# LoganWilliams1/mhm2_kmer_analysis_v2

Hardware: AMD Instinct MI355X
Metric: k-mers/sec (kcount stage) at k=21 (higher is better)
Workload: dtype u64

## Files before the change

### include/kcount_mi355.h

```cpp
#ifndef KCOUNT_MI355_H
#define KCOUNT_MI355_H

#include <stddef.h>
#include <stdint.h>

#ifdef __cplusplus
extern "C" {
#endif

#define KC_ABI_VERSION 1

enum {
  KC_OK = 0,
  KC_ERR_INVALID_ARG = -1,
  KC_ERR_UNSUPPORTED_K = -2,
  KC_ERR_NO_DEVICE = -3,
  KC_ERR_HIP = -4,
  KC_ERR_OUT_OF_MEMORY = -5,
  KC_ERR_CAPACITY = -6,
  KC_ERR_BAD_BASE = -7,
  KC_ERR_STATE = -8
};

typedef struct kc_ctx kc_ctx;
// ... 16 lines not shown
#define KC_FLAG_SHARD_BUCKETS 4u
#define KC_FLAG_WIRE_UNITS 8u
#define KC_FLAG_TIME_KERNELS 1u

typedef struct kc_stats {
  uint64_t num_reads;
  uint64_t num_bases;
  uint64_t raw_kmers;
  uint64_t kmers_inserted;
  uint64_t num_unique;
  uint64_t num_purged;
  uint64_t total_kmers;
  uint64_t sum_counts;
  uint64_t num_dropped;
  uint64_t capacity;
  uint64_t num_gpu_calls;
  uint64_t table_bytes;
} kc_stats;

typedef struct kc_result {
  uint64_t n;
  int32_t num_longs;
  int32_t reserved;
  const uint64_t *d_keys;
  const uint16_t *d_counts;
  const uint8_t *d_left;
  const uint8_t *d_right;
} kc_result;

int kc_abi_version(void);
const char *kc_error_string(int status);
const char *kc_last_error(void);
int kc_device_count(void);

int kc_num_longs(int kmer_len);
int kc_record_longs(int kmer_len);
int kc_owner(const uint64_t *kmer_words, int kmer_len, int rank_n);
int kc_owner_reference(const uint64_t *kmer_words, int kmer_len, int rank_n);

kc_ctx *kc_create(const kc_config *cfg, int *status);
void kc_destroy(kc_ctx *ctx);
int kc_set_stream(kc_ctx *ctx, void *hip_stream);
int kc_reset(kc_ctx *ctx, int new_kmer_len);

int kc_submit_reads(kc_ctx *ctx, const uint8_t *bases, const uint8_t *quals, const uint64_t *offsets, uint64_t nreads,
                    int on_device);

int kc_submit_packed_reads(kc_ctx *ctx, const uint8_t *packed, const uint64_t *offsets, uint64_t nreads, int on_device);

int kc_fastq_to_packed(const char *text, uint64_t len, int qual_offset, uint8_t *packed, uint64_t packed_capacity, uint64_t *offsets,
                       uint64_t reads_capacity, uint64_t *nreads, uint64_t *nbytes);

int kc_fastq_pairs(const char *text1, uint64_t len1, const char *text2, uint64_t len2, uint8_t *bases, uint8_t *quals,
                   uint64_t capacity, uint64_t *offsets, uint64_t reads_capacity, uint64_t *nreads, uint64_t *nbytes);

#define KC_FASTQ_PARTIAL 1u

int kc_fastq_to_packed_device(kc_ctx *ctx, const char *text, uint64_t len, int on_device, uint32_t flags, uint8_t *d_packed,
                              uint64_t packed_capacity, uint64_t *d_offsets, uint64_t reads_capacity, uint64_t *nreads,
                              uint64_t *nbytes, uint64_t *consumed);

int kc_fastq_pairs_device(kc_ctx *ctx, const char *text1, uint64_t len1, const char *text2, uint64_t len2, int on_device,
                          uint32_t flags, uint8_t *d_bases, uint8_t *d_quals, uint64_t capacity, uint64_t *d_offsets,
                          uint64_t reads_capacity, uint64_t *nreads, uint64_t *nbytes, uint64_t *consumed1, uint64_t *consumed2);

typedef struct kc_merge_stats {
// ... 132 lines not shown
```

### mhm2_kmer_analysis_v2_amd/_lib.py

```python
import ctypes as C
import os

_HERE = os.path.dirname(os.path.abspath(__file__))
_LIB = None

KC_OK = 0
KC_ERR_INVALID_ARG = -1
KC_ERR_CAPACITY = -6
KC_ERR_UNSUPPORTED_K = -2
KC_ERR_BAD_BASE = -7
KC_ERR_STATE = -8
KC_FLAG_TIME_KERNELS = 1
KC_FASTQ_PARTIAL = 1
KC_ADAPTERS_BLASTN_SCORES = 1
KC_TRIM_PAIRED = 1
KC_FLAG_REFERENCE_OWNER = 2
KC_FLAG_SHARD_BUCKETS = 4
KC_FLAG_WIRE_UNITS = 8


class KcError(RuntimeError):
    def __init__(self, status, where=""):
        self.status = status
        L = lib()
# ... 19 lines not shown
                ("d_counts", C.c_void_p), ("d_left", C.c_void_p), ("d_right", C.c_void_p)]


class kc_tuning(C.Structure):
    _fields_ = [("mode", C.c_uint32), ("writers", C.c_uint32), ("p1", C.c_uint32), ("p2", C.c_uint32), ("slots", C.c_uint32),
                ("chunk1", C.c_uint32), ("chunk2", C.c_uint32), ("chain1_max", C.c_uint32), ("chain2_max", C.c_uint32),
                ("arena1", C.c_uint32), ("ovf_capacity", C.c_uint64)]


class kc_kernel_time(C.Structure):
    _fields_ = [("name", C.c_char * 48), ("launches", C.c_uint64), ("total_ms", C.c_double)]


class kc_synth_params(C.Structure):
    _fields_ = [("seed", C.c_uint64), ("num_genomes", C.c_uint32), ("read_len", C.c_uint32), ("min_genome_len", C.c_uint64),
                ("max_genome_len", C.c_uint64), ("sub_error_rate", C.c_double), ("lowq_rate", C.c_double),
                ("n_rate", C.c_double), ("abundance_sigma", C.c_double)]


class kc_merge_stats(C.Structure):
    _fields_ = [(n, C.c_uint64) for n in ("pairs", "merged", "ambiguous", "dropped", "overlap_len", "merged_len", "out_reads",
                                           "out_bases")]


class kc_trim_stats(C.Structure):
    _fields_ = [(n, C.c_uint64) for n in ("reads", "trimmed", "bases_trimmed", "reads_removed", "alignments", "out_bases")]


SYMBOLS = {
    "kc_abi_version": (C.c_int, []),
    "kc_error_string": (C.c_char_p, [C.c_int]),
    "kc_last_error": (C.c_char_p, []),
    "kc_device_count": (C.c_int, []),
    "kc_num_longs": (C.c_int, [C.c_int]),
    "kc_record_longs": (C.c_int, [C.c_int]),
    "kc_owner": (C.c_int, [C.c_void_p, C.c_int, C.c_int]),
    "kc_owner_reference": (C.c_int, [C.c_void_p, C.c_int, C.c_int]),
    "kc_create": (C.c_void_p, [C.POINTER(kc_config), C.POINTER(C.c_int)]),
    "kc_destroy": (None, [C.c_void_p]),
    "kc_set_stream": (C.c_int, [C.c_void_p, C.c_void_p]),
    "kc_reset": (C.c_int, [C.c_void_p, C.c_int]),
    "kc_submit_reads": (C.c_int, [C.c_void_p, C.c_void_p, C.c_void_p, C.c_void_p, C.c_uint64, C.c_int]),
    "kc_submit_packed_reads": (C.c_int, [C.c_void_p, C.c_void_p, C.c_void_p, C.c_uint64, C.c_int]),
    "kc_fastq_to_packed": (C.c_int, [C.c_char_p, C.c_uint64, C.c_int, C.c_void_p, C.c_uint64, C.c_void_p, C.c_uint64, C.POINTER(C.c_uint64),
                                      C.POINTER(C.c_uint64)]),
    "kc_fastq_pairs": (C.c_int, [C.c_char_p, C.c_uint64, C.c_char_p, C.c_uint64, C.c_void_p, C.c_void_p, C.c_uint64, C.c_void_p,
                                  C.c_uint64, C.POINTER(C.c_uint64), C.POINTER(C.c_uint64)]),
    "kc_fastq_to_packed_device": (C.c_int, [C.c_void_p, C.c_void_p, C.c_uint64, C.c_int, C.c_uint32, C.c_void_p, C.c_uint64, C.c_void_p,
                                             C.c_uint64, C.POINTER(C.c_uint64), C.POINTER(C.c_uint64), C.POINTER(C.c_uint64)]),
    "kc_fastq_pairs_device": (C.c_int, [C.c_void_p, C.c_void_p, C.c_uint64, C.c_void_p, C.c_uint64, C.c_int, C.c_uint32, C.c_void_p,
                                         C.c_void_p, C.c_uint64, C.c_void_p, C.c_uint64, C.POINTER(C.c_uint64), C.POINTER(C.c_uint64),
                                         C.POINTER(C.c_uint64), C.POINTER(C.c_uint64)]),
    "kc_merge_pairs": (C.c_int, [C.c_void_p, C.c_void_p, C.c_void_p, C.c_void_p, C.c_uint64, C.c_int, C.c_int, C.c_void_p, C.c_uint64,
                                  C.c_void_p, C.c_uint64, C.POINTER(C.c_uint64), C.POINTER(C.c_uint64), C.POINTER(kc_merge_stats)]),
    "kc_adapters_index": (C.c_int, [C.c_char_p, C.c_uint64, C.c_int, C.POINTER(C.c_uint64), C.POINTER(C.c_uint64), C.POINTER(C.c_uint64),
                                     C.POINTER(C.c_uint64)]),
    "kc_adapters_load": (C.c_int, [C.c_void_p, C.c_char_p, C.c_uint64, C.c_int, C.c_uint32, C.POINTER(C.c_uint64), C.POINTER(C.c_uint64),
                                    C.POINTER(C.c_uint64), C.POINTER(C.c_uint64)]),
    "kc_adapters_clear": (C.c_int, [C.c_void_p]),
    "kc_trim_adapters": (C.c_int, [C.c_void_p, C.c_void_p, C.c_void_p, C.c_void_p, C.c_uint64, C.c_int, C.c_uint32, C.c_void_p, C.c_void_p,
                                    C.c_uint64, C.c_void_p, C.POINTER(C.c_uint64), C.POINTER(kc_trim_stats)]),
    "kc_submit_seq_block": (C.c_int, [C.c_void_p, C.c_void_p, C.c_uint64, C.c_int]),
    "kc_extract_partition": (C.c_int, [C.c_void_p, C.c_void_p, C.c_void_p, C.c_void_p, C.c_uint64, C.c_int, C.c_void_p,
                                       C.c_uint64, C.c_void_p]),
    "kc_extract_partition_seq_block": (C.c_int, [C.c_void_p, C.c_void_p, C.c_uint64, C.c_int, C.c_void_p, C.c_uint64, C.c_void_p]),
    "kc_insert_records": (C.c_int, [C.c_void_p, C.c_void_p, C.c_uint64]),
# ... 57 lines not shown
```

### mhm2_kmer_analysis_v2_amd/csrc/kc_api.hip

```cpp
#include <hip/hip_runtime.h>

#include <math.h>
#include <stdio.h>
#include <stdlib.h>
#include <string.h>

#include <algorithm>
#include <new>
#include <thread>
#include <string>
#include <type_traits>
#include <unordered_map>
#include <vector>

#include "../../include/kcount_mi355.h"
#include "kc_bucketed.hpp"
#include "kc_shard.hpp"
#include "kc_wire6.hpp"
#include "kc_supermer.hpp"
#include "kc_ctg.hpp"
#include "kc_merge.hpp"
#include "kc_trim.hpp"
#include "kc_fastq.hpp"

// ... 286 lines not shown

static int ensure_tile_first(kc_ctx *c, size_t ntiles) {
  if (ntiles <= c->tile_first_cap) return KC_OK;
  if (c->d_tile_first) HIPCHK(hipFree(c->d_tile_first));
  c->d_tile_first = nullptr;
  c->tile_first_cap = 0;
  HIPCHK(hipMalloc((void **)&c->d_tile_first, ntiles * 8));
  c->tile_first_cap = ntiles;
  return KC_OK;
}

static int table_insert_records(kc_ctx *c, const uint64_t *d_records, uint64_t n, uint32_t count_inserted) {
  uint64_t done = 0;
  while (done < n) {
    uint64_t m = std::min<uint64_t>(n - done, std::max<uint64_t>(c->capacity / 4, 1u << 18));
    int rc = ensure_room(c, m);
    if (rc) return rc;
    const uint64_t *p = d_records + done * c->nl;
    {
      KernelTimer kt(c, KT_INSERT_RECORDS);
      const unsigned nblk = (unsigned)std::min<uint64_t>((m + TPB - 1) / TPB, 256 * 32);
      with_nl(c, [&](auto nl) {
        hipLaunchKernelGGL(kc_insert_records_kernel<nl>, dim3(nblk), dim3(TPB), 0, c->stream, p, m, c->table, c->d_ctrs, count_inserted);
      });
    }
    HIPCHK(hipGetLastError());
    done += m;
  }
  return KC_OK;
}

extern "C" int kc_abi_version(void) { return KC_ABI_VERSION; }

extern "C" const char *kc_error_string(int s) {
  switch (s) {
    case KC_OK: return "ok";
    case KC_ERR_INVALID_ARG: return "invalid argument";
    case KC_ERR_UNSUPPORTED_K: return "unsupported k-mer length";
    case KC_ERR_NO_DEVICE: return "no usable HIP device";
    case KC_ERR_HIP: return "HIP call failed";
    case KC_ERR_OUT_OF_MEMORY: return "out of device memory";
    case KC_ERR_CAPACITY: return "a buffer is too small (kc_last_error says which)";
    case KC_ERR_BAD_BASE: return "read holds a byte outside ACGTN";
    case KC_ERR_STATE: return "call not allowed in this state";
    default: return "unknown status";
  }
}

extern "C" const char *kc_last_error(void) { return g_last_error; }

extern "C" int kc_device_count(void) {
  int n = 0;
  if (hipGetDeviceCount(&n) != hipSuccess) return 0;
  return n;
}

extern "C" int kc_num_longs(int k) { return k / 32 + 1; }

extern "C" int kc_record_longs(int k) { return k / 32 + 1 + ((k % 32) >= 30 ? 1 : 0); }

static int check_k(int k) {
  if (k < 3 || k > 127) return KC_ERR_UNSUPPORTED_K;
  if (kc_record_longs(k) > KC_MAX_LONGS) return KC_ERR_UNSUPPORTED_K;
  return KC_OK;
}

// ... 1073 lines not shown
  a.records = d_records;
  a.seg_capacity = seg_capacity;
  const int64_t end = (int64_t)a.align + (int64_t)total;
  bool over_capacity = false;
  if (mode == MODE_INSERT) {
    c->started = true;
    if (bk_active(c)) {
      int rc = bk_init(c);
      if (rc) return rc;
      uint64_t total;
      if (host_occ && c->expect_host_ok) {
        c->expect_host += *host_occ;
        total = c->expect_host;
      } else {
        rc = sync_ctrs(c);
        if (rc) return rc;
        if (c->h_ctrs[CTR_BAD_BASE]) return KC_ERR_BAD_BASE;
        total = c->h_ctrs[CTR_EXPECT];
        c->expect_host = total;
        c->expect_host_ok = true;
      }
      over_capacity = total - c->expect_base > c->bk_capacity;
      if (over_capacity && !c->sh.flow && c->expect_prev > c->expect_base && total - c->expect_prev <= c->bk_capacity) {
        rc = bk_make_room(c, c->expect_prev - c->expect_base);
        if (rc) return rc;
        c->expect_base = c->expect_prev;
        over_capacity = false;
      }
      c->expect_prev = total;
    } else {
      c->expect_host_ok = false;
    }
  }
  int64_t p0 = 0;
  while (p0 < end) {
    const bool bk = (mode == MODE_INSERT) && bk_active(c);
    const bool super = bk || mode == MODE_BIN;
    const uint64_t span = super ? (uint64_t)SUPER_SPAN : (uint64_t)TILE;
    uint64_t chunk_tiles;
    if (super) {
      chunk_tiles = (1ULL << 31) / span;
    } else {
      chunk_tiles = std::max<uint64_t>(64, (c->capacity / 4) / span);
      chunk_tiles = std::min<uint64_t>(chunk_tiles, (1ULL << 28) / span);
    }
    uint64_t nt = std::min<uint64_t>(chunk_tiles, ((uint64_t)(end - p0) + span - 1) / span);
    if (bk && over_capacity && c->sh.flow) {
      snprintf(g_last_error, sizeof(g_last_error), "shard flow: more k-mers than max_kmers_buffered (%llu): raise it, or use kc_extract_partition / kc_insert_records",
               (unsigned long long)c->bk_capacity);
      return KC_ERR_CAPACITY;
    }
    if (bk && over_capacity) {
      int rc = bk_drain_to_table(c);
      if (rc) return rc;
      continue;
    }
    if (bk) {
      uint64_t room = 0;
      int rc = bk_ovf1_room(c, nt * span, &room);
      if (rc) return rc;
      nt = std::max<uint64_t>(1, std::min<uint64_t>(nt, room / span));
      c->ovf1_ub += nt * span;
      if (room < span) {
        snprintf(g_last_error, sizeof(g_last_error), "overflow list smaller than one tile of %llu positions: raise ovf_capacity", (unsigned long long)span);
        return KC_ERR_CAPACITY;
      }
// ... 2495 lines not shown
```

### mhm2_kmer_analysis_v2_amd/csrc/kc_bucketed.hpp

```cpp
#pragma once
#include "kc_kernels.hpp"

namespace kc {

constexpr int WGB = 1024;
constexpr int SUPER_SPAN = 16 * WGB - PRE - POST;
using TileSuper = TileGeo<WGB, SUPER_SPAN>;
static_assert(TileSuper::GPT == 1 && TileSuper::NGROUP == WGB, "one group per thread");
constexpr int PMAX = 1024;
constexpr int GMAX = 512;

template <int NL> struct Rnd {
  static constexpr int RPOS = NL == 1 ? 16 : NL == 2 ? 8 : 4;
  static constexpr int RPOS_READS = NL == 1 ? 8 : NL <= 3 ? 4 : 2;
  static constexpr size_t STAGE = ((size_t)WGB * RPOS + 64) * NL * 8;
  static constexpr size_t STAGE_READS = ((size_t)WGB * RPOS_READS + 64) * NL * 8;
};

struct Geom {
  uint32_t G, P1, P2, S;
  uint32_t log2CH1, log2CH2;
  uint32_t L1MAX, L2MAX;
  uint32_t A1;
  uint32_t A2;
// ... 342 lines not shown
  D.arena = bb.rec1 + (((size_t)g * gm.A1) << gm.log2CH1) * NL;
  D.chain = bb.chain1 + (size_t)g * gm.P1 * gm.L1MAX;
  D.log2CH = gm.log2CH1;
  D.LMAX = gm.L1MAX;
  D.arena_cap = gm.A1;
  D.arena_base = 0;
  D.own_lo = gm.own_lo;
  D.own_hi = gm.own_hi;
  return D;
}

__device__ __forceinline__ ChainDest l1_dest6(const Geom &gm, const BucketBufs &bb, uint32_t g) {
  ChainDest D = l1_dest<1>(gm, bb, g);
  D.arena = reinterpret_cast<uint64_t *>(reinterpret_cast<uint8_t *>(bb.rec1) + (((size_t)g * gm.A1) << gm.log2CH1) * 6);
  return D;
}

template <int NL, bool CP>
__device__ __forceinline__ void l1_overflow(const Geom &gm, const BucketBufs &bb, uint64_t *cb, const uint64_t (&r)[NL]) {
  const uint64_t o = atomicAdd((unsigned long long *)&cb[CB_OVF1], 1ULL);
  if (o < bb.ovf1_cap) {
#pragma unroll
    for (int w = 0; w < NL; w++) bb.ovf1[o * NL + w] = (CP && w == 0) ? cp_unmix_rec(r[w], gm) : r[w];
  } else {
    atomicOr((unsigned long long *)&cb[CB_FATAL], (unsigned long long)FATAL_OVF1);
  }
}

template <int KT, int RPOS, bool SH, class TL>
__device__ __forceinline__ void cp_run_fixed(const TL &L, int lp0, bool active, const Geom &gm, const ExtractArgs &a, uint32_t (&lo)[RPOS],
                                             uint32_t (&bk)[RPOS]) {
  const int K = KT ? KT : (int)a.k;
  const int NB = RPOS + K + 1;
  static_assert(RPOS + KT + 1 <= 32 && RPOS % 8 == 0 && PRE % 8 == 0, "the window must fit one word and never start word-aligned");
  const uint64_t *W = reinterpret_cast<const uint64_t *>(L.codes);
  const uint32_t *OK = reinterpret_cast<const uint32_t *>(L.ok);
  const int p = lp0 - 1, q = p >> 5, s = p & 31;
  const uint64_t w0 = W[q], w1 = W[q + 1];
  const uint32_t ok0 = OK[q], ok1 = OK[q + 1], g0 = L.gap[q], g1 = L.gap[q + 1];
  const uint64_t Wn = (w0 << (2 * s)) | (w1 >> (64 - 2 * s));
  const uint32_t nok = ~__builtin_amdgcn_alignbit(ok1, ok0, (uint32_t)s);
  const uint32_t gapw = __builtin_amdgcn_alignbit(g1, g0, (uint32_t)s);
  const uint64_t Rn = kc_rc_word(Wn) << (64 - 2 * NB);
  const uint64_t MID = ((1ULL << (2 * K)) - 1ULL) << 2;
  const uint32_t MK = (1u << K) - 1u;
#pragma unroll
  for (int j = 0; j < RPOS; j++) {
    const uint64_t x = Wn >> (64 - 2 * (j + K + 2)), y = Rn >> (64 - 2 * (RPOS - 1 - j + K + 2));
    const uint64_t CMP = (K & 1) ? (MID | 3ULL) : MID;
    const bool swap = (y & CMP) < (x & CMP);
    const uint64_t sel = swap ? y : x;
    const uint32_t na = (nok >> j) & 1u, nb = (nok >> (j + K + 1)) & 1u;
    const uint32_t le = ((uint32_t)(sel >> (2 * K + 2)) & 3u) | ((swap ? nb : na) << 2);
    const uint32_t re = ((uint32_t)sel & 3u) | ((swap ? na : nb) << 2);
    uint32_t Lh = (uint32_t)(sel >> (K + 2)) & MK, Rh = (uint32_t)(sel >> 2) & MK;
    bool valid = active && ((gapw >> (j + 1)) & ((1u << (K + 1)) - 1u)) == 0u;
    if (SH) {
      uint64_t key[1] = {(((uint64_t)Lh << K) | Rh) << (64 - 2 * K)};
      const uint32_t owner = a.reference_owner ? 0u : kc_owner_of_hash(kc_hash<1>(key), a.rank_n);
      if (a.reference_owner) {
        uint64_t rk[1];
        kc_revcomp<1>(key, K, rk);
        valid = valid && kc_reference_owner<1>(key, rk, K, a.rank_n) == a.rank_me;
      } else {
        valid = valid && owner == a.rank_me;
      }
    }
    Lh ^= kc_feistel_f(Rh, 0, K);
    Rh ^= kc_feistel_f(Lh, 1, K);
    Lh ^= kc_feistel_f(Rh, 2, K);
    const uint64_t mix = ((uint64_t)Lh << K) | Rh;
    lo[j] = (uint32_t)mix;
    bk[j] = valid ? ((uint32_t)(mix >> (2 * K - gm.la)) | (le << 10) | (re << 13)) : ~0u;
// ... 112 lines not shown
          },
          br, D, cst);
      }
      if (round == NROUND - 1) {
        const uint64_t nst = work ? st + gridDim.x : st;
        tile_encode<FMT, TileSuper>(L.tile, raw, a, a.pos0 + (int64_t)nst * SUPER_SPAN, ctrs, tid, nst < nsuper);
        tile_prefetch<FMT, TileSuper>(raw, a, a.pos0 + (int64_t)(nst + gridDim.x) * SUPER_SPAN, tid, next_first, nst + gridDim.x < nsuper);
        next_first = first_of(nst + 2 * (uint64_t)gridDim.x);
        KC_SPLIT_STAMP(5)
      }
      if (work) {
        split_copy_out<NL>(
            L.sp, sorted, sbucket, total, D, [&](const uint64_t (&r)[NL]) { return cp_b1(r[0], gm); },
            [&](uint32_t, const uint64_t (&r)[NL]) { l1_overflow<NL, CP>(gm, bb, cb, r); },
            [&](size_t i, const uint64_t (&r)[NL]) { store_words<NL>(D.arena, i, r); });
        buf ^= 1;
      }
    }
  }
  if ((uint32_t)tid < P1) bb.cnt1[(size_t)g * P1 + tid] = cst.cur;
  if (tid == 0) {
    bb.used1[g] = min(L.sp.arena_used, gm.A1);
    bb.used1[gm.G + g] = min(L.sp.arena_top, gm.A1);
  }
  for (int o = 32; o > 0; o >>= 1) n_ins += __shfl_down(n_ins, o);
  if (lane_id() == 0 && n_ins) atomicAdd((unsigned long long *)&ctrs[CTR_INSERTED], (unsigned long long)n_ins);
}

constexpr int R16 = 16;
constexpr uint32_t ST16_MAIN = (uint32_t)WGB * R16 + PMAX;
constexpr uint32_t ST16_SLOTS = ST16_MAIN + 64;
static_assert(SUPER_SPAN % R16 == 0 && SUPER_SPAN / R16 <= WGB, "one run of sixteen positions per thread covers the super-tile");
static_assert(ST16_MAIN < 65536, "staging positions fit 16 bits");
constexpr size_t l1x16_lds_bytes() { return ((sizeof(L1LDS) + 15) & ~size_t(15)) + (size_t)ST16_SLOTS * 6; }

template <class MidFn>
__device__ __forceinline__ uint32_t split_stage_pairs(SplitLDS &L, uint32_t *slo, uint16_t *sbk, int buf, uint32_t P, const uint32_t (&lo)[R16],
                                                      const uint32_t (&br)[R16], const ChainDest &D, ChainState &st, MidFn mid) {
  const int tid = fresh_tid();
  KC_SPLIT_STAMP(1)
  const uint32_t v = ((uint32_t)tid < P) ? L.hist[buf][tid] : 0u;
  const uint32_t excl = block_excl_scan((v + 1u) & ~1u, L.scan);
  const uint32_t CHm = (1u << D.log2CH) - 1u;
  if ((uint32_t)tid < P) {
    const uint32_t base = st.cur;
    uint32_t fit = v;
    const uint64_t room = ((uint64_t)D.LMAX << D.log2CH) - base;
    if ((uint64_t)fit > room) fit = (uint32_t)room;
    const uint32_t have = (base + CHm) >> D.log2CH;
    uint32_t k = ((base + fit + CHm) >> D.log2CH) - have, a = 0;
    if (k) {
      const bool own = (uint32_t)tid >= D.own_lo && (uint32_t)tid < D.own_hi;
      if (own) {
        a = atomicAdd(&L.arena_used, k);
        const uint32_t left = D.arena_cap - min(D.arena_cap, L.arena_top);
        if (a + k > left) {
          k = a < left ? left - a : 0;
          const uint64_t cap = ((uint64_t)(have + k) << D.log2CH) - base;
          if ((uint64_t)fit > cap) fit = (uint32_t)cap;
        }
      } else {
        const uint32_t t = atomicAdd(&L.arena_top, k);
        const uint32_t left = D.arena_cap - min(D.arena_cap, L.arena_used);
        if (t + k > left) {
          k = 0;
          const uint64_t cap = ((uint64_t)have << D.log2CH) - base;
          if ((uint64_t)fit > cap) fit = (uint32_t)cap;
// ... 90 lines not shown
      }
      odd |= (real1 && !pair) || (live && !f0);
    }
    if (__any(odd)) {
#pragma unroll
      for (int u = 0; u < U; u++) {
        const uint32_t i = i0 + 2u * (uint32_t)u * WGB;
        if (i >= total) continue;
        const uint32_t j = i - (d[u].z & 0xFFFFu), v = d[u].z >> 16, fit = d[u].w & 0xFFFFu, wold = d[u].w >> 16;
        const uint32_t at0 = (j < wold ? d[u].x : d[u].y) + i, at1 = (j + 1u < wold ? d[u].x : d[u].y) + i + 1u;
        const uint32_t l0 = (uint32_t)lo2[u], l1 = (uint32_t)(lo2[u] >> 32);
        const uint64_t bh = (uint64_t)(bk2[u] & (PMAX - 1)) << shb;
        const uint64_t ra = bh | ((uint64_t)l0 << shl) | (uint64_t)((bk2[u] >> 10) & 63u);
        const uint64_t rb = bh | ((uint64_t)l1 << shl) | (uint64_t)(bk2[u] >> 26);
        const bool f0 = j < fit, real1 = j + 1u < v, f1 = real1 && j + 1u < fit;
        if (!f0) overflow(ra);
        if (real1 && !(f0 && f1 && at1 == at0 + 1u)) {
          if (f1) {
            Rec6 r;
            r.lo = l1;
            r.bk = (uint16_t)(bk2[u] >> 16);
            *reinterpret_cast<Rec6 *>(arena0 + (size_t)at1 * 6) = r;
          } else {
            overflow(rb);
          }
        }
      }
    }
  }
  KC_SPLIT_STAMP(4)
}

template <int FMT, bool SH, int KK>
__global__ __launch_bounds__(WGB) void kc_l1_reads16_kernel(ExtractArgs a, Geom gm, BucketBufs bb, uint64_t nsuper, uint32_t rot, uint64_t *ctrs,
                                                            uint64_t *cb) {
  extern __shared__ __align__(16) uint8_t smem[];
  L1LDS &L = *reinterpret_cast<L1LDS *>(smem);
  uint32_t *slo = reinterpret_cast<uint32_t *>(smem + ((sizeof(L1LDS) + 15) & ~size_t(15)));
  uint16_t *sbk = reinterpret_cast<uint16_t *>(slo + ST16_SLOTS);
  const int tid = threadIdx.x;
  const uint32_t g = (blockIdx.x + rot) % gm.G, P1 = gm.P1;
  ChainDest D = l1_dest6(gm, bb, g);
#ifdef KC_STAMPS
  unsigned long long tprev_ = __builtin_amdgcn_s_memtime();
  D.stamps = cb + 8;
  D.tprev = &tprev_;
#endif
  ChainState cst = split_load_state(L.sp, P1, bb.cnt1 + (size_t)g * P1, D.chain, D.LMAX, D.log2CH, bb.used1[g], bb.used1[gm.G + g]);
  __syncthreads();
  uint32_t n_ins = 0;
  int buf = 0;
  TileRaw<TileSuper> raw;
  auto first_of = [&](uint64_t st) -> uint64_t { return (FMT != FMT_SEQBLOCK && st < nsuper) ? a.tile_first[st] : 0; };
  tile_prefetch<FMT, TileSuper>(raw, a, a.pos0 + (int64_t)blockIdx.x * SUPER_SPAN, tid, first_of(blockIdx.x), blockIdx.x < nsuper);
  uint64_t next_first = first_of((uint64_t)blockIdx.x + gridDim.x);
  constexpr int RUNS = SUPER_SPAN / R16;
  {
    const int ft = fresh_tid();
    tile_encode<FMT, TileSuper>(L.tile, raw, a, a.pos0 + (int64_t)blockIdx.x * SUPER_SPAN, ctrs, ft, blockIdx.x < nsuper);
    tile_prefetch<FMT, TileSuper>(raw, a, a.pos0 + (int64_t)((uint64_t)blockIdx.x + gridDim.x) * SUPER_SPAN, ft, next_first,
                                  (uint64_t)blockIdx.x + gridDim.x < nsuper);
    next_first = first_of((uint64_t)blockIdx.x + 2 * (uint64_t)gridDim.x);
  }
  for (uint64_t st = blockIdx.x; st < nsuper; st += gridDim.x) {
    uint32_t lo[R16], br[R16];
    const bool active = tid < RUNS;
    const int lp0 = PRE + (active ? tid : 0) * R16;
    {
      uint32_t l8[8], b8[8];
// ... 10 lines not shown
        br[8 + j] = b8[j];
      }
    }
#pragma unroll
    for (int j = 0; j < R16; j++) {
      const bool valid = br[j] != ~0u;
      const uint32_t rank = hist_rank(L.sp, buf, br[j] & (PMAX - 1), valid);
      br[j] = valid ? (br[j] | (rank << 16)) : ~0u;
      n_ins += valid ? 1u : 0u;
    }
    KC_SPLIT_STAMP(0)
    lds_barrier();
    const int ft = fresh_tid();
    const uint64_t nst = st + gridDim.x;
    tile_encode_clear<TileSuper>(L.tile, raw, ft);
    const uint32_t total = split_stage_pairs(L.sp, slo, sbk, buf, P1, lo, br, D, cst, [&]() {
      tile_encode_fill<FMT, TileSuper>(L.tile, raw, a, a.pos0 + (int64_t)nst * SUPER_SPAN, ctrs, ft, nst < nsuper);
      tile_prefetch<FMT, TileSuper>(raw, a, a.pos0 + (int64_t)(nst + gridDim.x) * SUPER_SPAN, ft, next_first, nst + gridDim.x < nsuper);
      next_first = first_of(nst + 2 * (uint64_t)gridDim.x);
    });
    split_copy_out_pairs(L.sp, slo, sbk, total, D, gm, [&](uint64_t r) {
      const uint64_t rr[1] = {r};
      l1_overflow<1, true>(gm, bb, cb, rr);
    });
    buf ^= 1;
  }
  if ((uint32_t)tid < P1) bb.cnt1[(size_t)g * P1 + tid] = cst.cur;
  if (tid == 0) {
    bb.used1[g] = min(L.sp.arena_used, gm.A1);
    bb.used1[gm.G + g] = min(L.sp.arena_top, gm.A1);
  }
  for (int o = 32; o > 0; o >>= 1) n_ins += __shfl_down(n_ins, o);
  if (lane_id() == 0 && n_ins) atomicAdd((unsigned long long *)&ctrs[CTR_INSERTED], (unsigned long long)n_ins);
}

template <int NL, int R>
__device__ __forceinline__ void split_round_flat(SplitLDS &L, int buf, uint32_t P, const uint64_t (&rec)[R][NL], const uint32_t (&br)[R],
                                                 uint64_t *records, uint64_t seg_cap, uint64_t *cursors, uint64_t *overflow_flag) {
  const int tid = threadIdx.x;
  if ((uint32_t)tid < P) {
    const uint32_t v = L.hist[buf][tid];
    uint64_t base = 0;
    if (v) base = atomicAdd((unsigned long long *)&cursors[tid], (unsigned long long)v);
    const uint64_t room = base < seg_cap ? seg_cap - base : 0;
    uint4 d;
    d.x = (uint32_t)base;
    d.y = (uint32_t)(base >> 32);
    d.z = (uint64_t)v <= room ? v : (uint32_t)room;
    d.w = 0;
    L.dst[tid] = d;
    L.hist[buf ^ 1][tid] = 0;
  }
  lds_barrier();
#pragma unroll
  for (int j = 0; j < R; j++) {
    if (br[j] != ~0u) {
      const uint32_t b = br[j] & (PMAX - 1), rank = br[j] >> 10;
      const uint4 d = L.dst[b];
      if (rank < d.z) {
        uint64_t *o = records + ((uint64_t)b * seg_cap + (((uint64_t)d.y << 32) | d.x) + rank) * NL;
#pragma unroll
        for (int w = 0; w < NL; w++) o[w] = rec[j][w];
      } else {
        *overflow_flag = 1;
      }
    }
// ... 1525 lines not shown
```

### mhm2_kmer_analysis_v2_amd/csrc/kc_kernels.hpp

```cpp
#pragma once
#include "kc_common.hpp"

namespace kc {

constexpr int TPB = 256;
constexpr int PPT = 16;
constexpr int TILE = TPB * PPT;
constexpr int PRE = 32;
constexpr int POST = 192;
template <int THREADS_, int SPAN_>
struct TileGeo {
  static constexpr int THREADS = THREADS_;
  static constexpr int SPAN = SPAN_;
  static constexpr int LSPAN = PRE + SPAN_ + POST;
  static constexpr int NGROUP = LSPAN / 16;
  static constexpr int NWORD = LSPAN / 32;
  static constexpr int GPT = (NGROUP + THREADS_ - 1) / THREADS_;
  static_assert(LSPAN % 32 == 0, "staged span must be whole words");
};
using TileSmall = TileGeo<TPB, TILE>;

constexpr uint64_t KEY_EMPTY = ~0ULL;
constexpr uint64_t KEY_BUSY = ~0ULL - 1;
constexpr uint64_t KEY_NEVER = ~0ULL - 2;

enum { MODE_INSERT = 0, MODE_BIN = 1 };
enum { FMT_READS = 0, FMT_SEQBLOCK = 1, FMT_PACKED = 2, FMT_READS_UQ = 3 };
constexpr bool fmt_is_reads(int fmt) { return fmt == FMT_READS || fmt == FMT_READS_UQ; }

enum {
  CTR_ENTRIES = 0,
  CTR_INSERTED,
  CTR_BAD_BASE,
  CTR_OUT,
  CTR_PURGED,
  CTR_SUM_COUNTS,
  CTR_RAW_KMERS,
  CTR_EXPECT,
  CTR_OVERFLOW,
  CTR_BIN0,
  CTR_COUNT = CTR_BIN0 + 64
};

struct Table {
  uint64_t *keys;
  uint32_t *vals;
  uint64_t mask;
};

struct ExtractArgs {
  const uint8_t *bases;
  const uint8_t *quals;
  const uint64_t *offsets;
  const uint64_t *tile_first;
  uint64_t nreads;
  uint64_t total;
  uint32_t align;
  int64_t pos0;
  int k;
  int qual_cut;
  uint32_t rank_me, rank_n;
  uint32_t reference_owner;
  uint64_t *records;
  uint64_t seg_capacity;
};

__device__ __forceinline__ uint32_t lane_id() { return __lane_id(); }

__device__ __forceinline__ void sat_inc(uint32_t *p) {
  uint32_t old = atomicAdd(p, 1u);
  if (old >= 0x80000000u) atomicSub(p, 1u);
}

template <int NL>
__device__ __forceinline__ uint64_t table_slot(const Table &t, const uint64_t (&key)[NL], bool &is_new) {
  uint64_t slot = kc_hash<NL>(key) & t.mask;
  is_new = false;
  if constexpr (NL == 1) {
    for (;;) {
      uint64_t cur = t.keys[slot];
      if (cur == key[0]) break;
      if (cur == KEY_EMPTY) {
        uint64_t old = atomicCAS((unsigned long long *)&t.keys[slot], (unsigned long long)KEY_EMPTY,
                                 (unsigned long long)key[0]);
        if (old == KEY_EMPTY) { is_new = true; break; }
        if (old == key[0]) break;
      }
// ... 468 lines not shown
  for (int o = 32; o > 0; o >>= 1) n_ins += __shfl_down(n_ins, o);
  if (lane_id() == 0 && n_ins) atomicAdd((unsigned long long *)&ctrs[CTR_INSERTED], (unsigned long long)n_ins);
}

template <int NL>
__global__ __launch_bounds__(TPB) void kc_insert_records_kernel(const uint64_t *recs, uint64_t n, Table t, uint64_t *ctrs,
                                                                 uint32_t count_inserted) {
  const uint64_t stride = (uint64_t)gridDim.x * TPB;
  uint32_t n_ins = 0;
  for (uint64_t i = (uint64_t)blockIdx.x * TPB + threadIdx.x; i < n; i += stride) {
    uint64_t rec[NL];
#pragma unroll
    for (int j = 0; j < NL; j++) rec[j] = recs[i * NL + j];
    table_insert<NL>(t, rec, ctrs);
    n_ins++;
  }
  for (int o = 32; o > 0; o >>= 1) n_ins += __shfl_down(n_ins, o);
  if (count_inserted && lane_id() == 0 && n_ins) atomicAdd((unsigned long long *)&ctrs[CTR_INSERTED], (unsigned long long)n_ins);
}

__global__ void kc_tile_first_kernel(const uint64_t *offsets, uint64_t nreads, uint32_t align, int64_t pos0, uint32_t span, uint64_t ntiles,
                                     uint64_t *tile_first) {
  uint64_t i = (uint64_t)blockIdx.x * blockDim.x + threadIdx.x;
  if (i >= ntiles) return;
  int64_t T0 = pos0 + (int64_t)i * span - (int64_t)align;
  uint64_t lo = 0, hi = nreads + 1;
  while (lo < hi) {
    uint64_t mid = (lo + hi) >> 1;
    if ((int64_t)offsets[mid] < T0) lo = mid + 1; else hi = mid;
  }
  tile_first[i] = lo;
}

__global__ void kc_read_stats_kernel(const uint64_t *offsets, uint64_t nreads, int k, uint64_t *ctrs, uint32_t count_expect) {
  uint64_t acc = 0, exp = 0;
  const uint64_t stride = (uint64_t)gridDim.x * blockDim.x;
  for (uint64_t r = (uint64_t)blockIdx.x * blockDim.x + threadIdx.x; r < nreads; r += stride) {
    uint64_t len = offsets[r + 1] - offsets[r];
    if (len >= (uint64_t)k) acc += len - k + 1;
    if (len >= (uint64_t)k + 2) exp += len - k - 1;
  }
  for (int o = 32; o > 0; o >>= 1) {
    acc += __shfl_down(acc, o);
    exp += __shfl_down(exp, o);
  }
  __shared__ unsigned long long s_acc, s_exp;
  if (threadIdx.x == 0) s_acc = s_exp = 0;
  __syncthreads();
  if (lane_id() == 0) {
    if (acc) atomicAdd(&s_acc, (unsigned long long)acc);
    if (exp) atomicAdd(&s_exp, (unsigned long long)exp);
  }
  __syncthreads();
  if (threadIdx.x == 0) {
    if (s_acc) atomicAdd((unsigned long long *)&ctrs[CTR_RAW_KMERS], s_acc);
    if (count_expect && s_exp) atomicAdd((unsigned long long *)&ctrs[CTR_EXPECT], s_exp);
  }
}

constexpr uint64_t SEQSTAT_SPAN = 4096;
__global__ void kc_seqblock_stats_kernel(const uint8_t *seqs, uint64_t len, int k, uint64_t *ctrs, uint32_t count_expect) {
  const uint32_t lane = lane_id();
  const uint64_t nwaves = ((uint64_t)gridDim.x * blockDim.x) >> 6, wave0 = ((uint64_t)blockIdx.x * blockDim.x + threadIdx.x) >> 6;
  uint64_t acc = 0, exp = 0;
  for (uint64_t w = wave0; w * SEQSTAT_SPAN < len; w += nwaves) {
    const uint64_t lo = w * SEQSTAT_SPAN, hi = lo + SEQSTAT_SPAN < len ? lo + SEQSTAT_SPAN : len;
// ... 203 lines not shown
```

Measured before the change: 100.0 billion.

## Schedule level-1 read kernel by groups of sixteen k-mer starts instead of positions

Adds a device-side prefix scan over reads that counts groups of sixteen valid k-mer starts per read and emits, for each tile of 1024 groups, the first read and start position. The level-1 bucketing kernel for read formats now walks these dense group tiles, so threads no longer spend lanes on read boundaries and invalid tail positions. Reads that spill past a tile continue in a follow-up iteration. This adds three small scan kernels, a larger LDS footprint and more complex per-tile bookkeeping, with risk around continuation and boundary handling.

```diff
diff --git a/include/kcount_mi355.h b/include/kcount_mi355.h
--- a/include/kcount_mi355.h
+++ b/include/kcount_mi355.h
@@ -72,6 +72,8 @@
 const char *kc_error_string(int status);
 const char *kc_last_error(void);
 int kc_device_count(void);
+int kc_group_tiles_host(const uint64_t *offsets, uint64_t num_reads, int kmer_len, uint32_t align, uint64_t *tiles,
+                        uint64_t tile_cap, uint64_t *groups);
 
 int kc_num_longs(int kmer_len);
 int kc_record_longs(int kmer_len);
diff --git a/mhm2_kmer_analysis_v2_amd/_lib.py b/mhm2_kmer_analysis_v2_amd/_lib.py
--- a/mhm2_kmer_analysis_v2_amd/_lib.py
+++ b/mhm2_kmer_analysis_v2_amd/_lib.py
@@ -75,6 +75,7 @@
     "kc_error_string": (C.c_char_p, [C.c_int]),
     "kc_last_error": (C.c_char_p, []),
     "kc_device_count": (C.c_int, []),
+    "kc_group_tiles_host": (C.c_int, [C.c_void_p, C.c_uint64, C.c_int, C.c_uint32, C.c_void_p, C.c_uint64, C.POINTER(C.c_uint64)]),
     "kc_num_longs": (C.c_int, [C.c_int]),
     "kc_record_longs": (C.c_int, [C.c_int]),
     "kc_owner": (C.c_int, [C.c_void_p, C.c_int, C.c_int]),
diff --git a/mhm2_kmer_analysis_v2_amd/csrc/kc_api.hip b/mhm2_kmer_analysis_v2_amd/csrc/kc_api.hip
--- a/mhm2_kmer_analysis_v2_amd/csrc/kc_api.hip
+++ b/mhm2_kmer_analysis_v2_amd/csrc/kc_api.hip
@@ -342,6 +342,29 @@
 
 extern "C" int kc_abi_version(void) { return KC_ABI_VERSION; }
 
+extern "C" int kc_group_tiles_host(const uint64_t *offsets, uint64_t nreads, int k, uint32_t align, uint64_t *tiles, uint64_t tile_cap,
+                                   uint64_t *groups) {
+  if (!offsets || !groups || (!tiles && tile_cap) || k < 1) return KC_ERR_INVALID_ARG;
+  const uint64_t nb = (nreads + GRP_BLOCK_READS - 1) / GRP_BLOCK_READS;
+  std::vector<uint64_t> bsum(nb + 1, 0);
+  for (uint64_t b = 0; b < nb; b++) {
+    uint64_t s = 0;
+    for (uint64_t r = b * GRP_BLOCK_READS; r < std::min<uint64_t>(nreads, (b + 1) * GRP_BLOCK_READS); r++) s += grp_of_len(offsets[r + 1] - offsets[r], k);
+    bsum[b + 1] = bsum[b] + s;
+  }
+  *groups = bsum[nb];
+  if ((bsum[nb] + GRP_TILE - 1) / GRP_TILE > tile_cap) return KC_ERR_CAPACITY;
+  for (uint64_t b = 0; b < nb; b++) {
+    uint64_t P = bsum[b];
+    for (uint64_t r = b * GRP_BLOCK_READS; r < std::min<uint64_t>(nreads, (b + 1) * GRP_BLOCK_READS); r++) {
+      const uint64_t ng = grp_of_len(offsets[r + 1] - offsets[r], k);
+      if (ng) grp_emit_tiles(P, ng, r, offsets[r], align, tiles);
+      P += ng;
+    }
+  }
+  return KC_OK;
+}
+
 extern "C" const char *kc_error_string(int s) {
   switch (s) {
     case KC_OK: return "ok";
@@ -1481,6 +1504,41 @@
       c->expect_host_ok = false;
     }
   }
+  if (mode == MODE_INSERT && bk_active(c) && !over_capacity && c->nl == 1 && c->gm.rec6 && fmt != FMT_SEQBLOCK) {
+    const uint64_t ntiles = (total / 16 + nreads) / GRP_TILE + 1, nb = (nreads + GRP_BLOCK_READS - 1) / GRP_BLOCK_READS;
+    const uint64_t span = (uint64_t)GRP_TILE * 16;
+    int rc = ensure_tile_first(c, 2 * ntiles + nb + 1);
+    if (rc) return rc;
+    uint64_t *d_bsum = c->d_tile_first + 2 * ntiles;
+    {
+      KernelTimer kt(c, KT_TILE_FIRST);
+      hipLaunchKernelGGL(kc_grp_sums_kernel, dim3((unsigned)nb), dim3(GRP_BLOCK_THREADS), 0, c->stream, d_offsets, nreads, c->k, d_bsum);
+      hipLaunchKernelGGL(kc_grp_scan_kernel, dim3(1), dim3(1024), 0, c->stream, d_bsum, nb, d_bsum + nb);
+      hipLaunchKernelGGL(kc_grp_tiles_kernel, dim3((unsigned)nb), dim3(GRP_BLOCK_THREADS), 0, c->stream, d_offsets, nreads, c->k, a.align, d_bsum,
+                         c->d_tile_first);
+    }
+    c->num_gpu_calls += 2;
+    HIPCHK(hipGetLastError());
+    a.tile_first = c->d_tile_first;
+    a.grp_total = d_bsum + nb;
+    for (uint64_t t0 = 0; t0 < ntiles;) {
+      uint64_t nt = std::min<uint64_t>((1ULL << 31) / span, ntiles - t0), room = 0;
+      rc = bk_ovf1_room(c, nt * span, &room);
+      if (rc) return rc;
+      if (room < span) {
+        snprintf(g_last_error, sizeof(g_last_error), "overflow list smaller than one tile of %llu positions: raise ovf_capacity", (unsigned long long)span);
+        return KC_ERR_CAPACITY;
+      }
+      nt = std::min<uint64_t>(nt, room / span);
+      c->ovf1_ub += nt * span;
+      a.pos0 = (int64_t)t0;
+      rc = launch_l1_reads(c, a, nt, fmt);
+      if (rc) return rc;
+      HIPCHK(hipGetLastError());
+      t0 += nt;
+    }
+    return KC_OK;
+  }
   int64_t p0 = 0;
   while (p0 < end) {
     const bool bk = (mode == MODE_INSERT) && bk_active(c);
diff --git a/mhm2_kmer_analysis_v2_amd/csrc/kc_bucketed.hpp b/mhm2_kmer_analysis_v2_amd/csrc/kc_bucketed.hpp
--- a/mhm2_kmer_analysis_v2_amd/csrc/kc_bucketed.hpp
+++ b/mhm2_kmer_analysis_v2_amd/csrc/kc_bucketed.hpp
@@ -398,13 +398,13 @@
                                              uint32_t (&bk)[RPOS]) {
   const int K = KT ? KT : (int)a.k;
   const int NB = RPOS + K + 1;
-  static_assert(RPOS + KT + 1 <= 32 && RPOS % 8 == 0 && PRE % 8 == 0, "the window must fit one word and never start word-aligned");
+  static_assert(RPOS + KT + 1 <= 32 && RPOS % 8 == 0, "the window must fit one word");
   const uint64_t *W = reinterpret_cast<const uint64_t *>(L.codes);
   const uint32_t *OK = reinterpret_cast<const uint32_t *>(L.ok);
   const int p = lp0 - 1, q = p >> 5, s = p & 31;
   const uint64_t w0 = W[q], w1 = W[q + 1];
   const uint32_t ok0 = OK[q], ok1 = OK[q + 1], g0 = L.gap[q], g1 = L.gap[q + 1];
-  const uint64_t Wn = (w0 << (2 * s)) | (w1 >> (64 - 2 * s));
+  const uint64_t Wn = (w0 << (2 * s)) | ((w1 >> 1) >> (63 - 2 * s));
   const uint32_t nok = ~__builtin_amdgcn_alignbit(ok1, ok0, (uint32_t)s);
   const uint32_t gapw = __builtin_amdgcn_alignbit(g1, g0, (uint32_t)s);
   const uint64_t Rn = kc_rc_word(Wn) << (64 - 2 * NB);
@@ -583,7 +583,23 @@
 constexpr uint32_t ST16_SLOTS = ST16_MAIN + 64;
 static_assert(SUPER_SPAN % R16 == 0 && SUPER_SPAN / R16 <= WGB, "one run of sixteen positions per thread covers the super-tile");
 static_assert(ST16_MAIN < 65536, "staging positions fit 16 bits");
-constexpr size_t l1x16_lds_bytes() { return ((sizeof(L1LDS) + 15) & ~size_t(15)) + (size_t)ST16_SLOTS * 6; }
+
+constexpr int GRP_LSPAN = 24576;
+using TileGrp = TileGeo<WGB, GRP_LSPAN - PRE - POST>;
+static_assert(TileGrp::GPT == 2 && GRP_TILE == (uint32_t)WGB, "one group of starts per thread, two groups of bytes to stage");
+constexpr int GRP_LP_MAX = PRE + TileGrp::SPAN - 15;
+static_assert(GRP_LP_MAX + 71 <= TileGrp::LSPAN && GRP_LSPAN < 65536, "the cut stays inside the image; positions fit 16 bits");
+struct L1GLDS {
+  TileLDS<TileGrp> tile;
+  SplitLDS sp;
+  uint32_t gbits[WGB / 32];
+  uint16_t gstart[WGB];
+  uint32_t gsum[WGB / 64];
+  uint32_t nstage;
+  uint32_t cont_key;
+};
+constexpr size_t l1x16_lds_bytes() { return ((sizeof(L1GLDS) + 15) & ~size_t(15)) + (size_t)ST16_SLOTS * 6; }
+static_assert(sizeof(L1GLDS) >= sizeof(L1LDS) && l1x16_lds_bytes() <= 160 * 1024, "level 1 fits the LDS of a CU");
 
 template <class MidFn>
 __device__ __forceinline__ uint32_t split_stage_pairs(SplitLDS &L, uint32_t *slo, uint16_t *sbk, int buf, uint32_t P, const uint32_t (&lo)[R16],
@@ -740,9 +756,8 @@
 }
 
 template <int FMT, bool SH, int KK>
-__global__ __launch_bounds__(WGB) void kc_l1_reads16_kernel(ExtractArgs a, Geom gm, BucketBufs bb, uint64_t nsuper, uint32_t rot, uint64_t *ctrs,
-                                                            uint64_t *cb) {
-  extern __shared__ __align__(16) uint8_t smem[];
+__device__ __forceinline__ void l1_reads16_positions(uint8_t *smem, const ExtractArgs &a, const Geom &gm, const BucketBufs &bb, uint64_t nsuper,
+                                                     uint32_t rot, uint64_t *ctrs, uint64_t *cb) {
   L1LDS &L = *reinterpret_cast<L1LDS *>(smem);
   uint32_t *slo = reinterpret_cast<uint32_t *>(smem + ((sizeof(L1LDS) + 15) & ~size_t(15)));
   uint16_t *sbk = reinterpret_cast<uint16_t *>(slo + ST16_SLOTS);
@@ -819,6 +834,210 @@
   }
   for (int o = 32; o > 0; o >>= 1) n_ins += __shfl_down(n_ins, o);
   if (lane_id() == 0 && n_ins) atomicAdd((unsigned long long *)&ctrs[CTR_INSERTED], (unsigned long long)n_ins);
+}
+
+struct GrpStage {
+  uint64_t r0;
+  int64_t s0;
+  uint32_t glim;
+  bool on;
+  __device__ __forceinline__ int64_t T0() const { return (s0 - 1) & ~(int64_t)15; }
+};
+struct GrpRead {
+  int fs;
+  uint32_t ngr, ng;
+};
+__device__ __forceinline__ GrpRead grp_read(const GrpStage &sg, const ExtractArgs &a, int tid, uint64_t off, uint32_t off1_lo) {
+  GrpRead g;
+  g.fs = PRE;
+  g.ngr = g.ng = 0;
+  if (sg.on && sg.r0 + (uint64_t)tid < a.nreads && off != ~0ULL) {
+    const int64_t rs = (int64_t)off + (int64_t)a.align;
+    const int64_t len = (int64_t)(uint32_t)(off1_lo - (uint32_t)off);
+    const int64_t fs = tid == 0 ? sg.s0 : rs + 1;
+    const int64_t nstarts = rs + len - (int64_t)a.k - fs;
+    const int64_t lp = fs - (sg.T0() - PRE);
+    if (nstarts > 0 && lp <= GRP_LP_MAX) {
+      g.fs = (int)lp;
+      g.ngr = (uint32_t)((nstarts + 15) >> 4);
+      g.ng = min(g.ngr, (uint32_t)((GRP_LP_MAX - (int)lp) >> 4) + 1u);
+    } else if (nstarts > 0) {
+      g.ngr = 1;
+    }
+  }
+  return g;
+}
+
+template <int FMT, bool SH, int KK>
+__device__ __forceinline__ void l1_reads16_groups(uint8_t *smem, const ExtractArgs &a, const Geom &gm, const BucketBufs &bb, uint64_t nsuper,
+                                                  uint32_t rot, uint64_t *ctrs, uint64_t *cb) {
+  L1GLDS &L = *reinterpret_cast<L1GLDS *>(smem);
+  uint32_t *slo = reinterpret_cast<uint32_t *>(smem + ((sizeof(L1GLDS) + 15) & ~size_t(15)));
+  uint16_t *sbk = reinterpret_cast<uint16_t *>(slo + ST16_SLOTS);
+  const int tid = threadIdx.x;
+  const uint32_t g = (blockIdx.x + rot) % gm.G, P1 = gm.P1;
+  ChainDest D = l1_dest6(gm, bb, g);
+#ifdef KC_STAMPS
+  unsigned long long tprev_ = __builtin_amdgcn_s_memtime();
+  D.stamps = cb + 8;
+  D.tprev = &tprev_;
+#endif
+  ChainState cst = split_load_state(L.sp, P1, bb.cnt1 + (size_t)g * P1, D.chain, D.LMAX, D.log2CH, bb.used1[g], bb.used1[gm.G + g]);
+  if (tid < WGB / 32) L.gbits[tid] = 0;
+  if (tid == 0) L.cont_key = ~0u;
+  __syncthreads();
+  uint32_t n_ins = 0;
+  int buf = 0;
+  const uint64_t gtot = *a.grp_total;
+  const uint64_t tend = min((uint64_t)a.pos0 + nsuper, (gtot + GRP_TILE - 1) / GRP_TILE);
+  auto tile_entry = [&](uint64_t t, uint64_t &r, uint64_t &s) {
+    r = t < tend ? a.tile_first[2 * t] : 0;
+    s = t < tend ? a.tile_first[2 * t + 1] : 1;
+  };
+  auto tile_stage = [&](uint64_t t, uint64_t r, uint64_t s) {
+    GrpStage sg;
+    sg.on = t < tend;
+    sg.r0 = r;
+    sg.s0 = (int64_t)s;
+    sg.glim = sg.on ? (uint32_t)min((uint64_t)GRP_TILE, gtot - t * GRP_TILE) : 0u;
+    return sg;
+  };
+  TileRaw<TileGrp> raw;
+  uint32_t off1_lo = 0;
+  auto prefetch = [&](const GrpStage &sg, int t) {
+    tile_prefetch<FMT, TileGrp>(raw, a, sg.T0(), t, sg.r0, sg.on);
+    off1_lo = 0;
+    if (sg.on && sg.r0 + (uint64_t)t + 1 <= a.nreads) off1_lo = (uint32_t)a.offsets[sg.r0 + (uint64_t)t + 1];
+  };
+  auto table_begin = [&](const GrpStage &sg, int t) -> uint32_t {
+    tile_encode_clear<TileGrp>(L.tile, raw, t);
+    if (t < WGB / 32) L.gbits[t] = 0;
+    if (t == 0) L.cont_key = ~0u;
+    const uint32_t incl = wave_incl_scan(grp_read(sg, a, t, raw.off, off1_lo).ng);
+    if (lane_id() == 63) L.gsum[t >> 6] = incl;
+    return incl;
+  };
+  auto table_finish = [&](const GrpStage &sg, int t, uint32_t incl) {
+    tile_encode_fill<FMT, TileGrp>(L.tile, raw, a, sg.T0(), ctrs, t, sg.on);
+    const GrpRead gr = grp_read(sg, a, t, raw.off, off1_lo);
+    const uint32_t w = lane_id() < WGB / 64 ? L.gsum[lane_id()] : 0u;
+    uint32_t wi = w;
+    wi += (uint32_t)__builtin_amdgcn_update_dpp(0, (int)wi, 0x111, 0xF, 0xF, false);
+    wi += (uint32_t)__builtin_amdgcn_update_dpp(0, (int)wi, 0x112, 0xF, 0xF, false);
+    wi += (uint32_t)__builtin_amdgcn_update_dpp(0, (int)wi, 0x114, 0xF, 0xF, false);
+    wi += (uint32_t)__builtin_amdgcn_update_dpp(0, (int)wi, 0x118, 0xF, 0xF, false);
+    const int wave = __builtin_amdgcn_readfirstlane(t >> 6);
+    const uint32_t first = incl - gr.ng + (uint32_t)__builtin_amdgcn_readlane((int)(wi - w), wave);
+    const uint32_t total = (uint32_t)__builtin_amdgcn_readlane((int)wi, WGB / 64 - 1);
+    if (gr.ng && first < (uint32_t)WGB) {
+      atomicOr(&L.gbits[first >> 5], 1u << (first & 31u));
+      L.gstart[first] = (uint16_t)gr.fs;
+    }
+    const bool unfinished = gr.ng < gr.ngr;
+    const uint64_t um = __ballot(unfinished);
+    if (unfinished && (um & ((1ULL << lane_id()) - 1ULL)) == 0) atomicMin(&L.cont_key, ((uint32_t)t << 16) | gr.ng);
+    if (t == 0) L.nstage = min(total, sg.glim);
+  };
+  uint64_t st = (uint64_t)a.pos0 + blockIdx.x, nn_r, nn_s;
+  tile_entry(st, nn_r, nn_s);
+  GrpStage cur = tile_stage(st, nn_r, nn_s);
+  {
+    const int ft = fresh_tid();
+    prefetch(cur, ft);
+    const uint32_t incl = table_begin(cur, ft);
+    tile_barrier();
+    table_finish(cur, ft, incl);
+    tile_barrier();
+  }
+  tile_entry(st + gridDim.x, nn_r, nn_s);
+  GrpStage nx = tile_stage(st + gridDim.x, nn_r, nn_s);
+  prefetch(nx, fresh_tid());
+  tile_entry(st + 2 * (uint64_t)gridDim.x, nn_r, nn_s);
+  while (cur.on) {
+    const uint32_t nstage = (uint32_t)__builtin_amdgcn_readfirstlane((int)L.nstage);
+    const uint32_t key = (uint32_t)__builtin_amdgcn_readfirstlane((int)L.cont_key);
+    uint32_t lo[R16], br[R16];
+    const bool active = (uint32_t)tid < nstage;
+    int lp0 = PRE;
+    if (active) {
+      int w = tid >> 5;
+      uint32_t m = L.gbits[w] & (0xFFFFFFFFu >> (31 - (tid & 31)));
+      while (m == 0u && w > 0) m = L.gbits[--w];
+      const int first = 32 * w + 31 - __builtin_clz(m | 1u);
+      lp0 = (int)L.gstart[first] + 16 * (tid - first);
+      lp0 = min(max(lp0, 1), GRP_LP_MAX);
+    }
+    {
+      uint32_t l8[8], b8[8];
+      cp_run_fixed<KK, 8, SH>(L.tile, lp0, active, gm, a, l8, b8);
+#pragma unroll
+      for (int j = 0; j < 8; j++) {
+        lo[j] = l8[j];
+        br[j] = b8[j];
+      }
+      cp_run_fixed<KK, 8, SH>(L.tile, lp0 + 8, active, gm, a, l8, b8);
+#pragma unroll
+      for (int j = 0; j < 8; j++) {
+        lo[8 + j] = l8[j];
+        br[8 + j] = b8[j];
+      }
+    }
+#pragma unroll
+    for (int j = 0; j < R16; j++) {
+      const bool valid = br[j] != ~0u;
+      const uint32_t rank = hist_rank(L.sp, buf, br[j] & (PMAX - 1), valid);
+      br[j] = valid ? (br[j] | (rank << 16)) : ~0u;
+      n_ins += valid ? 1u : 0u;
+    }
+    KC_SPLIT_STAMP(0)
+    lds_barrier();
+    const int ft = fresh_tid();
+    GrpStage nd = nx;
+    uint64_t nst = st + gridDim.x;
+    const bool cont = nstage < cur.glim;
+    if (cont) {
+      const uint32_t t = key >> 16;
+      nd.r0 = cur.r0 + (key == ~0u ? (uint32_t)WGB : t);
+      nd.glim = cur.glim - nstage;
+      nd.on = nd.r0 < a.nreads;
+      nd.s0 = 1;
+      if (nd.on) nd.s0 = (key != ~0u && t == 0u ? cur.s0 : (int64_t)a.offsets[nd.r0] + (int64_t)a.align + 1) + (key == ~0u ? 0 : 16 * (int64_t)(key & 0xFFFFu));
+      nst = st;
+      prefetch(nd, ft);
+    }
+    const uint32_t incl = table_begin(nd, ft);
+    const uint32_t total = split_stage_pairs(L.sp, slo, sbk, buf, P1, lo, br, D, cst, [&]() {
+      table_finish(nd, ft, incl);
+      if (!cont) nx = tile_stage(nst + gridDim.x, nn_r, nn_s);
+      prefetch(nx, ft);
+      if (!cont) tile_entry(nst + 2 * (uint64_t)gridDim.x, nn_r, nn_s);
+    });
+    split_copy_out_pairs(L.sp, slo, sbk, total, D, gm, [&](uint64_t r) {
+      const uint64_t rr[1] = {r};
+      l1_overflow<1, true>(gm, bb, cb, rr);
+    });
+    buf ^= 1;
+    cur = nd;
+    st = nst;
+  }
+  if ((uint32_t)tid < P1) bb.cnt1[(size_t)g * P1 + tid] = cst.cur;
+  if (tid == 0) {
+    bb.used1[g] = min(L.sp.arena_used, gm.A1);
+    bb.used1[gm.G + g] = min(L.sp.arena_top, gm.A1);
+  }
+  for (int o = 32; o > 0; o >>= 1) n_ins += __shfl_down(n_ins, o);
+  if (lane_id() == 0 && n_ins) atomicAdd((unsigned long long *)&ctrs[CTR_INSERTED], (unsigned long long)n_ins);
+}
+
+template <int FMT, bool SH, int KK>
+__global__ __launch_bounds__(WGB) void kc_l1_reads16_kernel(ExtractArgs a, Geom gm, BucketBufs bb, uint64_t nsuper, uint32_t rot, uint64_t *ctrs,
+                                                            uint64_t *cb) {
+  extern __shared__ __align__(16) uint8_t smem[];
+  if constexpr (FMT == FMT_SEQBLOCK) {
+    l1_reads16_positions<FMT, SH, KK>(smem, a, gm, bb, nsuper, rot, ctrs, cb);
+  } else {
+    l1_reads16_groups<FMT, SH, KK>(smem, a, gm, bb, nsuper, rot, ctrs, cb);
+  }
 }
 
 template <int NL, int R>
diff --git a/mhm2_kmer_analysis_v2_amd/csrc/kc_kernels.hpp b/mhm2_kmer_analysis_v2_amd/csrc/kc_kernels.hpp
--- a/mhm2_kmer_analysis_v2_amd/csrc/kc_kernels.hpp
+++ b/mhm2_kmer_analysis_v2_amd/csrc/kc_kernels.hpp
@@ -53,6 +53,7 @@
   const uint8_t *quals;
   const uint64_t *offsets;
   const uint64_t *tile_first;
+  const uint64_t *grp_total;
   uint64_t nreads;
   uint64_t total;
   uint32_t align;
@@ -587,6 +588,89 @@
   tile_first[i] = lo;
 }
 
+constexpr uint32_t GRP_TILE = 1024;
+constexpr uint32_t GRP_BLOCK_THREADS = 256, GRP_READS_PER_THREAD = 8;
+constexpr uint32_t GRP_BLOCK_READS = GRP_BLOCK_THREADS * GRP_READS_PER_THREAD;
+__host__ __device__ inline uint64_t grp_of_len(uint64_t len, int k) { return len > (uint64_t)k + 1 ? (len - (uint64_t)k - 1 + 15) >> 4 : 0; }
+__host__ __device__ inline void grp_emit_tiles(uint64_t P, uint64_t ng, uint64_t read, uint64_t off, uint32_t align, uint64_t *tiles) {
+  for (uint64_t i = (P + GRP_TILE - 1) / GRP_TILE; i * GRP_TILE < P + ng; i++) {
+    tiles[2 * i] = read;
+    tiles[2 * i + 1] = off + align + 1 + 16 * (i * GRP_TILE - P);
+  }
+}
+
+__device__ __forceinline__ uint64_t grp_thread_counts(const uint64_t *offsets, uint64_t nreads, int k, uint64_t r0, uint64_t (&o)[GRP_READS_PER_THREAD],
+                                                      uint64_t (&ng)[GRP_READS_PER_THREAD]) {
+  uint64_t sum = 0, prev = r0 < nreads ? offsets[r0] : 0;
+#pragma unroll
+  for (uint32_t j = 0; j < GRP_READS_PER_THREAD; j++) {
+    o[j] = prev;
+    ng[j] = 0;
+    if (r0 + j < nreads) {
+      const uint64_t nxt = offsets[r0 + j + 1];
+      ng[j] = grp_of_len(nxt - prev, k);
+      prev = nxt;
+    }
+    sum += ng[j];
+  }
+  return sum;
+}
+
+__device__ __forceinline__ uint64_t grp_block_scan(uint64_t v, uint64_t *wsum, uint64_t *total) {
+  uint64_t x = v;
+  for (int o = 1; o < 64; o <<= 1) {
+    const uint64_t y = __shfl_up(x, o);
+    if ((int)lane_id() >= o) x += y;
+  }
+  const uint32_t wave = threadIdx.x >> 6, nw = blockDim.x >> 6;
+  if (lane_id() == 63) wsum[wave] = x;
+  __syncthreads();
+  uint64_t pre = 0, tot = 0;
+  for (uint32_t w = 0; w < nw; w++) {
+    if (w < wave) pre += wsum[w];
+    tot += wsum[w];
+  }
+  __syncthreads();
+  *total = tot;
+  return pre + x - v;
+}
+
+__global__ __launch_bounds__(GRP_BLOCK_THREADS) void kc_grp_sums_kernel(const uint64_t *offsets, uint64_t nreads, int k, uint64_t *bsum) {
+  __shared__ uint64_t wsum[16];
+  uint64_t o[GRP_READS_PER_THREAD], ng[GRP_READS_PER_THREAD], tot;
+  const uint64_t s = grp_thread_counts(offsets, nreads, k, (uint64_t)blockIdx.x * GRP_BLOCK_READS + (uint64_t)threadIdx.x * GRP_READS_PER_THREAD, o, ng);
+  grp_block_scan(s, wsum, &tot);
+  if (threadIdx.x == 0) bsum[blockIdx.x] = tot;
+}
+
+__global__ __launch_bounds__(1024) void kc_grp_scan_kernel(uint64_t *bsum, uint64_t nb, uint64_t *total) {
+  __shared__ uint64_t wsum[16];
+  uint64_t carry = 0;
+  for (uint64_t base = 0; base < nb; base += 1024) {
+    const uint64_t i = base + threadIdx.x;
+    const uint64_t v = i < nb ? bsum[i] : 0;
+    uint64_t tot;
+    const uint64_t ex = grp_block_scan(v, wsum, &tot);
+    if (i < nb) bsum[i] = carry + ex;
+    carry += tot;
+  }
+  if (threadIdx.x == 0) *total = carry;
+}
+
+__global__ __launch_bounds__(GRP_BLOCK_THREADS) void kc_grp_tiles_kernel(const uint64_t *offsets, uint64_t nreads, int k, uint32_t align,
+                                                                         const uint64_t *bsum, uint64_t *tiles) {
+  __shared__ uint64_t wsum[16];
+  uint64_t o[GRP_READS_PER_THREAD], ng[GRP_READS_PER_THREAD], tot;
+  const uint64_t r0 = (uint64_t)blockIdx.x * GRP_BLOCK_READS + (uint64_t)threadIdx.x * GRP_READS_PER_THREAD;
+  const uint64_t s = grp_thread_counts(offsets, nreads, k, r0, o, ng);
+  uint64_t P = bsum[blockIdx.x] + grp_block_scan(s, wsum, &tot);
+#pragma unroll
+  for (uint32_t j = 0; j < GRP_READS_PER_THREAD; j++) {
+    if (ng[j]) grp_emit_tiles(P, ng[j], r0 + j, o[j], align, tiles);
+    P += ng[j];
+  }
+}
+
 __global__ void kc_read_stats_kernel(const uint64_t *offsets, uint64_t nreads, int k, uint64_t *ctrs, uint32_t count_expect) {
   uint64_t acc = 0, exp = 0;
   const uint64_t stride = (uint64_t)gridDim.x * blockDim.x;
```

Measured after the change: 99.90 billion (median of 2 runs). No clear change (-0.1%).
